# BOpermanis/SP-SLAM

Measured on AMD Instinct MI355X. Metric: RGB-D frames/sec (track+planes+poseOpt) at 640x480; ATE vs CPU ref, higher is better.
Workload: dtype u8+f32+f64

## Files before the change

### sp-slam_amd/csrc/libm64_cr.h

```cpp
#pragma once
#if defined(__HIP__)
#include <hip/hip_runtime.h>
#define SPSLAM_CR_TABLE(T, name, dims) __device__ constexpr T name dims
#else
#ifndef __host__
#define __host__
#endif
#ifndef __device__
#define __device__
#endif
#include <cmath>
#define SPSLAM_CR_TABLE(T, name, dims) constexpr T name dims
#endif

namespace spslam {
namespace libm64cr {

#include "libm64_cr_tables.inc"

struct dd { double hi, lo; };

__host__ __device__ inline dd two_sum(double a, double b) {
    const double s = a + b, bb = s - a;
    return {s, (a - (s - bb)) + (b - bb)};
}
__host__ __device__ inline dd fast_two_sum(double a, double b) {
    const double s = a + b;
    return {s, b - (s - a)};
}
__host__ __device__ inline dd dmul(dd a, dd b) {
    const double p = a.hi * b.hi;
    double e = fma(a.hi, b.hi, -p);
    e = fma(a.hi, b.lo, e);
    e = fma(a.lo, b.hi, e);
    return fast_two_sum(p, e);
}
__host__ __device__ inline dd dmul_d(dd a, double b) {
    const double p = a.hi * b;
    double e = fma(a.hi, b, -p);
    e = fma(a.lo, b, e);
    return fast_two_sum(p, e);
}
__host__ __device__ inline dd dadd(dd a, dd b) {
    const dd s = two_sum(a.hi, b.hi);
    return fast_two_sum(s.hi, s.lo + (a.lo + b.lo));
}
__host__ __device__ inline dd dadd_d(dd a, double b) {
    const dd s = two_sum(a.hi, b);
    return fast_two_sum(s.hi, s.lo + a.lo);
}
__host__ __device__ inline dd dneg(dd a) { return {-a.hi, -a.lo}; }
__host__ __device__ inline dd ddiv(dd a, dd b) {
    const double q1 = a.hi / b.hi;
    const dd r = dadd(a, dneg(dmul_d(b, q1)));
    return fast_two_sum(q1, r.hi / b.hi);
}
__host__ __device__ inline dd ddiv_r(dd a, dd b) {
    const double r = 1.0 / b.hi;
    const double q1 = a.hi * r;
    const dd rem = dadd(a, dneg(dmul_d(b, q1)));
    return fast_two_sum(q1, rem.hi * r);
}

__host__ __device__ inline bool rounds_to(dd r, double eps, double* out) {
    const double e = eps * fabs(r.hi);
    const double a = r.hi + (r.lo - e), b = r.hi + (r.lo + e);
    *out = a;
    return a == b;
}

constexpr double kQuickEps = 0x1p-70;
constexpr double kAccurateEps = 0x1p-98;

template <bool kAccurate>
__host__ __device__ inline void sin_cm1(dd t, dd* s, dd* cm1) {
    const dd t2 = dmul(t, t);
    if (!kAccurate) {
        const double q = t2.hi;
        const double ps = kSinC[2][0] + q * (kSinC[3][0] + q * (kSinC[4][0] + q * kSinC[5][0]));
        const dd P = dadd_d(dd{kSinC[1][0], kSinC[1][1]}, q * ps);
        *s = dadd(t, dmul(dmul(t, t2), P));
        const double pc = kCosC[2][0] + q * (kCosC[3][0] + q * (kCosC[4][0] + q * kCosC[5][0]));
        *cm1 = dadd(dd{-0.5 * t2.hi, -0.5 * t2.lo}, dd{q * (q * pc), 0.0});
    } else {
        dd P{kSinC[11][0], kSinC[11][1]}, C{kCosC[11][0], kCosC[11][1]};
        for (int k = 10; k >= 1; k--) {
            P = dadd(dmul(P, t2), dd{kSinC[k][0], kSinC[k][1]});
            C = dadd(dmul(C, t2), dd{kCosC[k][0], kCosC[k][1]});
        }
        *s = dadd(t, dmul(dmul(t, t2), P));
        *cm1 = dmul(t2, C);
    }
}

template <bool kAccurate>
__host__ __device__ inline void sincos_reduced(dd r, dd* s, dd* c) {
    const double jf = rint(r.hi * 64.0);
    const int j = (int)jf;
    const dd t = two_sum(r.hi - jf * 0.015625, r.lo);
    dd st, cm1;
    sin_cm1<kAccurate>(t, &st, &cm1);
    const int aj = (int)fmin(fabs(jf), 64.0);
    const double sg = j < 0 ? -1.0 : 1.0;
    const dd S{sg * kSinCos64[aj][0], sg * kSinCos64[aj][1]}, C{kSinCos64[aj][2], kSinCos64[aj][3]};
    *s = dadd(S, dadd(dmul(S, cm1), dmul(C, st)));
    *c = dadd(C, dadd(dmul(C, cm1), dneg(dmul(S, st))));
}

__host__ __device__ inline dd reduce_pio2(double x, int* k) {
    const double kf = rint(x * kInvPio2);
    *k = (int)(kf - 4.0 * floor(kf * 0.25));
    const double ph = kf * kPio2_1, pl = fma(kf, kPio2_1, -ph);
    const double qh = kf * kPio2_2, ql = fma(kf, kPio2_2, -qh);
    const dd a = two_sum(x - ph, -qh);
    const dd b = two_sum(a.hi, -pl);
    return fast_two_sum(b.hi, ((a.lo + b.lo) - ql) - kf * kPio2_3);
}

template <bool kAccurate>
__host__ __device__ inline void sincos_eval(double x, dd* s, dd* c) {
    int k;
    const dd r = reduce_pio2(x, &k);
    dd sr, cr;
    sincos_reduced<kAccurate>(r, &sr, &cr);
    const int n = k & 3;
    const dd a = (n & 1) ? cr : sr, b = (n & 1) ? sr : cr;
    *s = (n & 2) ? dneg(a) : a;
    *c = ((n + 1) & 2) ? dneg(b) : b;
}

#if defined(__HIP__)
#define SPSLAM_CR_COLD __attribute__((noinline))
#else
#define SPSLAM_CR_COLD
#endif
__host__ __device__ SPSLAM_CR_COLD inline dd sincos_accurate(double x) {
    dd s, c;
    sincos_eval<true>(x, &s, &c);
    double rs, rc;
    rounds_to(s, kAccurateEps, &rs);
    rounds_to(c, kAccurateEps, &rc);
    return dd{rs, rc};
}

__host__ __device__ inline bool sincos_quick(double x, double* sn, double* cs) {
    const double ax = fabs(x);
    const bool nonfinite = !(ax <= 1.7976931348623157e308);
    const bool tiny = ax < 0x1p-27;
    const bool special = nonfinite || tiny;
    dd s, c;
    sincos_eval<false>(special ? 1.0 : x, &s, &c);
    double rs, rc;
    const bool ok_s = rounds_to(s, kQuickEps, &rs), ok_c = rounds_to(c, kQuickEps, &rc);
    *sn = nonfinite ? x - x : (tiny ? x : rs);
    *cs = nonfinite ? x - x : (tiny ? 1.0 : rc);
    return special || (ok_s && ok_c);
}

__host__ __device__ inline void sincos_(double x, double* sn, double* cs) {
    if (!sincos_quick(x, sn, cs)) {
        const dd a = sincos_accurate(x);
        *sn = a.hi;
        *cs = a.lo;
    }
}
__host__ __device__ inline void sincos2_(double x0, double x1, double* s0, double* c0, double* s1, double* c1) {
    const bool ok0 = sincos_quick(x0, s0, c0), ok1 = sincos_quick(x1, s1, c1);
    if (!(ok0 && ok1)) {
        if (!ok0) { const dd a = sincos_accurate(x0); *s0 = a.hi; *c0 = a.lo; }
        if (!ok1) { const dd a = sincos_accurate(x1); *s1 = a.hi; *c1 = a.lo; }
    }
}
__host__ __device__ inline double sin_(double x) {
    double s, c;
    sincos_(x, &s, &c);
    return s;
}
__host__ __device__ inline double cos_(double x) {
    double s, c;
    sincos_(x, &s, &c);
    return c;
}

template <bool kAccurate>
__host__ __device__ inline dd atan_small(dd u) {
    const dd u2 = dmul(u, u);
    dd P;
    if (!kAccurate) {
        const double q = u2.hi;
        const double pa = kAtanC[2][0] +
                          q * (kAtanC[3][0] + q * (kAtanC[4][0] + q * (kAtanC[5][0] + q * (kAtanC[6][0] + q * kAtanC[7][0]))));
        P = dadd_d(dd{kAtanC[1][0], kAtanC[1][1]}, q * pa);
    } else {
        P = dd{kAtanC[11][0], kAtanC[11][1]};
        for (int k = 10; k >= 1; k--) P = dadd(dmul(P, u2), dd{kAtanC[k][0], kAtanC[k][1]});
    }
    return dadd(u, dmul(dmul(u, u2), P));
}

template <bool kAccurate>
__host__ __device__ inline dd atan2_eval(double y, double x) {
    const double ax = fabs(x), ay = fabs(y);
    const bool swap = ay > ax;
    const double num = swap ? ax : ay, den = swap ? ay : ax;
    double zh, zl;
    if (kAccurate) {
        zh = num / den;
        zl = fma(-zh, den, num) / den;
    } else {
        const double rd = 1.0 / den;
        zh = num * rd;
        zl = fma(-zh, den, num) * rd;
    }
    const dd z{zh, zl};
    const double fi = rint(zh * 64.0);
    const int i = (int)fi;
    const double c = fi * 0.015625;
    const dd nm = two_sum(zh - c, z.lo);
    const dd dn = dadd_d(dmul_d(z, c), 1.0);
    const dd uq = kAccurate ? ddiv(nm, dn) : ddiv_r(nm, dn);
    const dd u{i == 0 ? z.hi : uq.hi, i == 0 ? z.lo : uq.lo};
    dd a = dadd(dd{kAtan64[i][0], kAtan64[i][1]}, atan_small<kAccurate>(u));
    const dd a1 = dadd(dd{kPio2_hi, kPio2_lo}, dneg(a));
    a = dd{swap ? a1.hi : a.hi, swap ? a1.lo : a.lo};
    const dd a2 = dadd(dd{kPi_hi, kPi_lo}, dneg(a));
    a = dd{x < 0 ? a2.hi : a.hi, x < 0 ? a2.lo : a.lo};
    return dd{y < 0 ? -a.hi : a.hi, y < 0 ? -a.lo : a.lo};
}

__host__ __device__ SPSLAM_CR_COLD inline double atan2_accurate(double y, double x) {
    if (!__builtin_signbit(x) && fabs(y) < fabs(x) * 0x1p-900) return y / x;
    double out;
    rounds_to(atan2_eval<true>(y, x), kAccurateEps, &out);
    return out;
}

__host__ __device__ inline bool atan2_quick(double y, double x, double* out) {
    const double ax = fabs(x), ay = fabs(y);
    const double inf = 1.7976931348623157e308 * 2.0;
    const double sy = __builtin_signbit(y) ? -1.0 : 1.0;
    const bool xneg = __builtin_signbit(x);
    const bool nan = x != x || y != y;
    const bool zy = ay == 0, zx = ax == 0, infs = ax == inf || ay == inf;
    const bool small = !xneg && ay < ax * 0x1p-900;
    const bool special = nan || zy || zx || infs;
    double sp = 0.0;
    if (infs) sp = ax == inf && ay == inf ? sy * (xneg ? k3Pio4_hi : kPio4_hi)
                                          : (ax == inf ? (xneg ? sy * kPi_hi : sy * 0.0) : sy * kPio2_hi);
    if (zx) sp = sy * kPio2_hi;
    if (zy) sp = xneg ? sy * kPi_hi : y;
    if (nan) sp = x + y;
    const double den = ax > ay ? ax : ay;
    const bool extreme = !(den >= 0x1p-1000 && den <= 0x1p1000);
    const bool stand_in = special || small || extreme;
    const dd r = atan2_eval<false>(stand_in ? 1.0 : y, stand_in ? 1.0 : x);
    double q;
    const bool ok = rounds_to(r, kQuickEps, &q) && !small && !extreme;
    *out = special ? sp : q;
    return special || ok;
}

__host__ __device__ inline double atan2_(double y, double x) {
    double out;
    if (!atan2_quick(y, x, &out)) out = atan2_accurate(y, x);
    return out;
}
__host__ __device__ inline void atan2x2_(double y0, double x0, double y1, double x1, double* r0, double* r1) {
    const bool ok0 = atan2_quick(y0, x0, r0), ok1 = atan2_quick(y1, x1, r1);
    if (!(ok0 && ok1)) {
        if (!ok0) *r0 = atan2_accurate(y0, x0);
        if (!ok1) *r1 = atan2_accurate(y1, x1);
    }
}

__host__ __device__ inline double cube_(double x) {
    const double h = x * x;
    const double l = fma(x, x, -h);
    const double p = h * x;
    const double e = fma(h, x, -p);
    if (x == 0 || !(fabs(p) <= 1.7976931348623157e308)) return p;
    return p + (e + l * x);
}

}
}
```

Measured before the change: 44490.

## Add cheaper first-stage sincos and atan2 evaluators ahead of quick/accurate paths

Adds a new stage-1 evaluator for sincos and atan2. It uses mostly double arithmetic with a table lookup (kSinCos64, kAtan64) and short polynomials, and checks the result against a looser 2^-64 rounding test. Only when that test fails does the code fall back to the existing double-double quick path and then the accurate path, with a compile macro choosing whether stage 2 is inlined or kept out of line. The aim is to cut the per-call cost of correctly rounded transcendentals in the tracking and pose kernels. In exchange, inputs that fail stage 1 pay extra work, and code size and register pressure grow.

```diff
diff --git a/sp-slam_amd/csrc/libm64_cr.h b/sp-slam_amd/csrc/libm64_cr.h
--- a/sp-slam_amd/csrc/libm64_cr.h
+++ b/sp-slam_amd/csrc/libm64_cr.h
@@ -71,6 +71,15 @@
 
 constexpr double kQuickEps = 0x1p-70;
 constexpr double kAccurateEps = 0x1p-98;
+
+constexpr double kStage1Eps = 0x1p-64;
+
+#ifndef SPSLAM_CR_DECLINE_STAGES
+#define SPSLAM_CR_DECLINE_STAGES 0
+#endif
+#ifndef SPSLAM_CR_STAGE2_INLINE
+#define SPSLAM_CR_STAGE2_INLINE 1
+#endif
 
 template <bool kAccurate>
 __host__ __device__ inline void sin_cm1(dd t, dd* s, dd* cm1) {
@@ -129,12 +138,47 @@
     *c = ((n + 1) & 2) ? dneg(b) : b;
 }
 
+__host__ __device__ inline bool sincos_eval1(double x, dd* s, dd* c) {
+    int k;
+    const dd r = reduce_pio2(x, &k);
+    const double jf = rint(r.hi * 64.0);
+    const dd t = fast_two_sum(r.hi - jf * 0.015625, r.lo);
+    const double th = t.hi, tl = t.lo;
+    const double t2h = th * th;
+    const double t2l = fma(th + th, tl, fma(th, th, -t2h));
+    const double ps = fma(t2h, fma(t2h, kSinC[3][0], kSinC[2][0]), kSinC[1][0]);
+    const double sl = (th * t2h) * ps + fma(-0.5 * tl, t2h, tl);
+    const double pc = fma(t2h, kCosC[3][0], kCosC[2][0]);
+    const double cmh = -0.5 * t2h;
+    const double cml = fma(t2h * t2h, pc, -0.5 * t2l);
+    const int aj = (int)fmin(fabs(jf), 64.0);
+    const double sg = jf < 0 ? -1.0 : 1.0;
+    const double Sh = sg * kSinCos64[aj][0], Sl = sg * kSinCos64[aj][1], Ch = kSinCos64[aj][2], Cl = kSinCos64[aj][3];
+    const double p1 = Ch * th, p2 = Sh * cmh;
+    const double e1 = fma(Ch, sl, fma(Cl, th, fma(Ch, th, -p1)));
+    const double e2 = fma(Sh, cml, fma(Sl, cmh, fma(Sh, cmh, -p2)));
+    const dd ws = two_sum(p1, p2);
+    const dd vs = fast_two_sum(Sh, ws.hi);
+    const dd sr{vs.hi, vs.lo + (ws.lo + (Sl + (e1 + e2)))};
+    const double p3 = Ch * cmh, p4 = Sh * th;
+    const double e3 = fma(Ch, cml, fma(Cl, cmh, fma(Ch, cmh, -p3)));
+    const double e4 = fma(Sh, sl, fma(Sl, th, fma(Sh, th, -p4)));
+    const dd wc = two_sum(p3, -p4);
+    const dd vc = fast_two_sum(Ch, wc.hi);
+    const dd cr{vc.hi, vc.lo + (wc.lo + (Cl + (e3 - e4)))};
+    const int n = k & 3;
+    const dd a = (n & 1) ? cr : sr, b = (n & 1) ? sr : cr;
+    *s = (n & 2) ? dneg(a) : a;
+    *c = ((n + 1) & 2) ? dneg(b) : b;
+    return fabs(r.hi) >= 0x1p-40;
+}
+
 #if defined(__HIP__)
 #define SPSLAM_CR_COLD __attribute__((noinline))
 #else
 #define SPSLAM_CR_COLD
 #endif
-__host__ __device__ SPSLAM_CR_COLD inline dd sincos_accurate(double x) {
+__host__ __device__ inline dd sincos_accurate_body(double x) {
     dd s, c;
     sincos_eval<true>(x, &s, &c);
     double rs, rc;
@@ -142,6 +186,7 @@
     rounds_to(c, kAccurateEps, &rc);
     return dd{rs, rc};
 }
+__host__ __device__ SPSLAM_CR_COLD inline dd sincos_accurate(double x) { return sincos_accurate_body(x); }
 
 __host__ __device__ inline bool sincos_quick(double x, double* sn, double* cs) {
     const double ax = fabs(x);
@@ -154,21 +199,47 @@
     const bool ok_s = rounds_to(s, kQuickEps, &rs), ok_c = rounds_to(c, kQuickEps, &rc);
     *sn = nonfinite ? x - x : (tiny ? x : rs);
     *cs = nonfinite ? x - x : (tiny ? 1.0 : rc);
-    return special || (ok_s && ok_c);
+    return special || (ok_s && ok_c && SPSLAM_CR_DECLINE_STAGES < 2);
+}
+
+__host__ __device__ inline bool sincos_stage1(double x, double* sn, double* cs) {
+    const double ax = fabs(x);
+    const bool nonfinite = !(ax <= 1.7976931348623157e308);
+    const bool tiny = ax < 0x1p-27;
+    const bool special = nonfinite || tiny;
+    dd s, c;
+    const bool in = sincos_eval1(special ? 1.0 : x, &s, &c) && ax < 0x1p20;
+    double rs, rc;
+    const bool ok_s = rounds_to(s, kStage1Eps, &rs), ok_c = rounds_to(c, kStage1Eps, &rc);
+    *sn = nonfinite ? x - x : (tiny ? x : rs);
+    *cs = nonfinite ? x - x : (tiny ? 1.0 : rc);
+    return special || (in && ok_s && ok_c && SPSLAM_CR_DECLINE_STAGES < 1);
+}
+
+__host__ __device__ SPSLAM_CR_COLD inline dd sincos_tail(double x) {
+    double s, c;
+    if (sincos_quick(x, &s, &c)) return dd{s, c};
+    return sincos_accurate_body(x);
+}
+__host__ __device__ inline void sincos_later(double x, double* sn, double* cs) {
+#if SPSLAM_CR_STAGE2_INLINE & 1
+    if (sincos_quick(x, sn, cs)) return;
+    const dd a = sincos_accurate(x);
+#else
+    const dd a = sincos_tail(x);
+#endif
+    *sn = a.hi;
+    *cs = a.lo;
 }
 
 __host__ __device__ inline void sincos_(double x, double* sn, double* cs) {
-    if (!sincos_quick(x, sn, cs)) {
-        const dd a = sincos_accurate(x);
-        *sn = a.hi;
-        *cs = a.lo;
-    }
+    if (!sincos_stage1(x, sn, cs)) sincos_later(x, sn, cs);
 }
 __host__ __device__ inline void sincos2_(double x0, double x1, double* s0, double* c0, double* s1, double* c1) {
-    const bool ok0 = sincos_quick(x0, s0, c0), ok1 = sincos_quick(x1, s1, c1);
+    const bool ok0 = sincos_stage1(x0, s0, c0), ok1 = sincos_stage1(x1, s1, c1);
     if (!(ok0 && ok1)) {
-        if (!ok0) { const dd a = sincos_accurate(x0); *s0 = a.hi; *c0 = a.lo; }
-        if (!ok1) { const dd a = sincos_accurate(x1); *s1 = a.hi; *c1 = a.lo; }
+        if (!ok0) sincos_later(x0, s0, c0);
+        if (!ok1) sincos_later(x1, s1, c1);
     }
 }
 __host__ __device__ inline double sin_(double x) {
@@ -228,14 +299,47 @@
     return dd{y < 0 ? -a.hi : a.hi, y < 0 ? -a.lo : a.lo};
 }
 
-__host__ __device__ SPSLAM_CR_COLD inline double atan2_accurate(double y, double x) {
+__host__ __device__ inline double atan2_accurate_body(double y, double x) {
     if (!__builtin_signbit(x) && fabs(y) < fabs(x) * 0x1p-900) return y / x;
     double out;
     rounds_to(atan2_eval<true>(y, x), kAccurateEps, &out);
     return out;
 }
-
-__host__ __device__ inline bool atan2_quick(double y, double x, double* out) {
+__host__ __device__ SPSLAM_CR_COLD inline double atan2_accurate(double y, double x) { return atan2_accurate_body(y, x); }
+
+__host__ __device__ inline dd atan2_eval1(double y, double x) {
+    const double ax = fabs(x), ay = fabs(y);
+    const bool swap = ay > ax;
+    const double num = swap ? ax : ay, den = swap ? ay : ax;
+    const double rd = 1.0 / den;
+    const double zh = num * rd, zl = fma(-zh, den, num) * rd;
+    const double fi = rint(zh * 64.0);
+    const int i = (int)fi;
+    const double c = fi * 0.015625;
+    const dd nm = two_sum(zh - c, zl);
+    const double p = zh * c;
+    const dd dn = fast_two_sum(1.0, p);
+    const double dl = dn.lo + fma(zl, c, fma(zh, c, -p));
+    const double rr = 1.0 / dn.hi;
+    const double q = nm.hi * rr;
+    const double ql = ((fma(-q, dn.hi, nm.hi) + nm.lo) - q * dl) * rr;
+    const double uh = i == 0 ? zh : q, ul = i == 0 ? zl : ql;
+    const double q2 = uh * uh;
+    const double P = fma(q2, fma(q2, fma(q2, kAtanC[4][0], kAtanC[3][0]), kAtanC[2][0]), kAtanC[1][0]);
+    const double t = (uh * q2) * P + fma(-ul, q2, ul);
+    const dd s0 = fast_two_sum(kAtan64[i][0], uh);
+    dd a{s0.hi, s0.lo + (kAtan64[i][1] + t)};
+    const dd s1 = fast_two_sum(kPio2_hi, -a.hi);
+    const double l1 = s1.lo + (kPio2_lo - a.lo);
+    a = dd{swap ? s1.hi : a.hi, swap ? l1 : a.lo};
+    const dd s2 = fast_two_sum(kPi_hi, -a.hi);
+    const double l2 = s2.lo + (kPi_lo - a.lo);
+    a = dd{x < 0 ? s2.hi : a.hi, x < 0 ? l2 : a.lo};
+    return dd{y < 0 ? -a.hi : a.hi, y < 0 ? -a.lo : a.lo};
+}
+
+struct atan2_args { double sp; bool special, slow; };
+__host__ __device__ inline atan2_args atan2_classify(double y, double x) {
     const double ax = fabs(x), ay = fabs(y);
     const double inf = 1.7976931348623157e308 * 2.0;
     const double sy = __builtin_signbit(y) ? -1.0 : 1.0;
@@ -243,7 +347,6 @@
     const bool nan = x != x || y != y;
     const bool zy = ay == 0, zx = ax == 0, infs = ax == inf || ay == inf;
     const bool small = !xneg && ay < ax * 0x1p-900;
-    const bool special = nan || zy || zx || infs;
     double sp = 0.0;
     if (infs) sp = ax == inf && ay == inf ? sy * (xneg ? k3Pio4_hi : kPio4_hi)
                                           : (ax == inf ? (xneg ? sy * kPi_hi : sy * 0.0) : sy * kPio2_hi);
@@ -252,24 +355,55 @@
     if (nan) sp = x + y;
     const double den = ax > ay ? ax : ay;
     const bool extreme = !(den >= 0x1p-1000 && den <= 0x1p1000);
-    const bool stand_in = special || small || extreme;
+    return atan2_args{sp, nan || zy || zx || infs, small || extreme};
+}
+
+__host__ __device__ inline bool atan2_stage1(double y, double x, double* out) {
+    const atan2_args k = atan2_classify(y, x);
+    const bool stand_in = k.special || k.slow;
+    const dd r = atan2_eval1(stand_in ? 1.0 : y, stand_in ? 1.0 : x);
+    double q;
+    const bool in = fmin(fabs(x), fabs(y)) >= 0x1p-960;
+    const bool ok = rounds_to(r, kStage1Eps, &q) && !k.slow && in && SPSLAM_CR_DECLINE_STAGES < 1;
+    *out = k.special ? k.sp : q;
+    return k.special || ok;
+}
+
+__host__ __device__ inline bool atan2_quick(double y, double x, double* out) {
+    const atan2_args k = atan2_classify(y, x);
+    const bool stand_in = k.special || k.slow;
     const dd r = atan2_eval<false>(stand_in ? 1.0 : y, stand_in ? 1.0 : x);
     double q;
-    const bool ok = rounds_to(r, kQuickEps, &q) && !small && !extreme;
-    *out = special ? sp : q;
-    return special || ok;
+    const bool ok = rounds_to(r, kQuickEps, &q) && !k.slow && SPSLAM_CR_DECLINE_STAGES < 2;
+    *out = k.special ? k.sp : q;
+    return k.special || ok;
+}
+
+__host__ __device__ SPSLAM_CR_COLD inline double atan2_tail(double y, double x) {
+    double out;
+    if (atan2_quick(y, x, &out)) return out;
+    return atan2_accurate_body(y, x);
+}
+__host__ __device__ inline double atan2_later(double y, double x) {
+#if SPSLAM_CR_STAGE2_INLINE & 2
+    double out;
+    if (atan2_quick(y, x, &out)) return out;
+    return atan2_accurate(y, x);
+#else
+    return atan2_tail(y, x);
+#endif
 }
 
 __host__ __device__ inline double atan2_(double y, double x) {
     double out;
-    if (!atan2_quick(y, x, &out)) out = atan2_accurate(y, x);
+    if (!atan2_stage1(y, x, &out)) out = atan2_later(y, x);
     return out;
 }
 __host__ __device__ inline void atan2x2_(double y0, double x0, double y1, double x1, double* r0, double* r1) {
-    const bool ok0 = atan2_quick(y0, x0, r0), ok1 = atan2_quick(y1, x1, r1);
+    const bool ok0 = atan2_stage1(y0, x0, r0), ok1 = atan2_stage1(y1, x1, r1);
     if (!(ok0 && ok1)) {
-        if (!ok0) *r0 = atan2_accurate(y0, x0);
-        if (!ok1) *r1 = atan2_accurate(y1, x1);
+        if (!ok0) *r0 = atan2_later(y0, x0);
+        if (!ok1) *r1 = atan2_later(y1, x1);
     }
 }
 
```

Result: no change. 44390 (-0.2%).
